# AechPro/rlgym-ppo

Hardware: AMD Instinct MI355X
Metric: ppo_update_samples_per_sec (higher is better)
Workload: dtype f32; 1 GPU; configs[1]: 4096 agents x 128 steps = 524,288-sample buffer, obs 107 f32, 90 discrete actions, 256x3 policy + critic; batch 524,288, minibatch 65,536

## Files before the change

### rlgym_ppo_amd/csrc/api.hip

```cpp
#include "build_id.h"
#include <math.h>
#include <stdarg.h>
#include <string.h>

#include "chain.hpp"

namespace rlppo {

static thread_local char g_err[512] = "";

void set_error(const char *fmt, ...) {
    va_list ap;
    va_start(ap, fmt);
    vsnprintf(g_err, sizeof(g_err), fmt, ap);
    va_end(ap);
}

static int64_t padded_width(int64_t d) {
    const int64_t p16 = round_up(d, 16), p64 = round_up(d, 64);
    return (p64 - p16) * 10 >= p64 ? p16 : p64;
}
static int64_t padded_out(int64_t d) {
    if (d <= 32) return 32;
    if (d <= 64) return 64;
// ... 709 lines not shown
int rlppo_dbg_set(int32_t key, int32_t value) {
    ++g_selection_epoch;
    switch (key) {
        case 1: set_gae_algo(value); return 0;
        case 4: set_two_streams(value); return 0;
        case 19: set_relu_bits(value); return 0;
        case 21: set_gae_spin_limit(value); return 0;
        case 22: set_gae_oversubscribe(value); return 0;
        case 34: set_fused_spin_limit(value); return 0;
        case 35: set_fused_test_hold(value); return 0;
        case 36: set_split_persistent(value); return 0;
        case 23: set_b16_wide_tiles(value); return 0;
        case 24: set_exp_fast_transform(value); return 0;
        case 26: set_fused_gather(value); return 0;
        case 27: g_fused_act = value; return 0;
        case 29: set_paired(value); return 0;
        case 31: set_head_order(value); return 0;
        case 32: set_fold_vhead(value); return 0;
        case 33: set_pair_interleave(value); return 0;
        case 37: set_group_dw(value); return 0;
        case 38: set_tn_group_budget(value); return 0;
        case 40: set_nt_skinny(value); return 0;
        case 41: g_window_mode = value; return 0;
        default: break;
    }
    set_error("dbg_set: unknown key %d", key);
    return RLPPO_ERR_ARG;
}
int64_t rlppo_selection_epoch(void) { return g_selection_epoch; }
const int64_t *rlppo_selection_epoch_ptr(void) { return &g_selection_epoch; }
int rlppo_dbg_count(int32_t key, int64_t delta) {
    RLPPO_CHECK_ARG(key == 6, "dbg_count: key %d (only counter 6 is kept by hosts that replay)", key);
    g_call_counts[CNT_MD_NVEC] += delta;
    return 0;
}
int64_t rlppo_dbg_counter(int32_t key) {
    switch (key) {
        case 0: case 1: case 2: case 3: case 4: case 5: case 6: return g_call_counts[key];
        case 7: return rollout_record_count();
        case 8: case 9: case 10: case 11: case 12: case 13: return g_form_launches[key - 8];
        case 15: return g_call_counts[CNT_CRITIC_ROWS_PASS];
        default: return -1;
    }
}
}
```

### rlgym_ppo_amd/csrc/chain.hip

```cpp
#include "chain.hpp"

namespace rlppo {

int max_pout(const NetLayout &net) {
    int m = 0;
    for (int l = 0; l < net.n_layers; ++l) m = net.L[l].pout > m ? net.L[l].pout : m;
    return m;
}

void x3_layout(const NetLayout &net, X3Layout *o) {
    int64_t off = 0;
    const int last = net.n_layers - 1;
    for (int l = 0; l < net.n_layers; ++l) {
        const LayerLayout &L = net.L[l];
        o->fwd[l] = o->dx[l] = -1;
        if (l >= 1 && l < last && nt_split_ok(L.pout, L.pin)) {
            o->fwd[l] = off;
            off += (int64_t)3 * L.pout * L.pin;
        }
        if (l >= 1 && !(l == last && gemv_head_ok(L.out, L.pin)) && nt_split_ok(L.pin, L.pout)) {
            o->dx[l] = off;
            off += (int64_t)3 * L.pin * L.pout;
        }
    }
// ... 166 lines not shown
            c.f32_valid[l] = true;
        }
        if (rc) return rc;
        x = acts[l];
        xb = actsb[l];
        x_f32 = c.f32_valid[l];
        ldx = L.pout;
    }
    return 0;
}

int layer_backward(Chain &c, int l, bool need_bits) {
    const NetLayout &net = *c.net;
    const int last = net.n_layers - 1;
    const LayerLayout &L = net.L[l];
    const hipStream_t st = c.st;
    const int64_t mb = c.n;
    float *const *acts = c.b.act, *const *dx = c.b.dx;
    const float *dY = l == last ? acts[last] : dx[l];
    const int64_t ld_hy = c.head_folded ? 1 : L.pout;
    const RowSource X = l > 0 ? RowSource{acts[l - 1], net.L[l - 1].pout} : c.in;
    const bool gemv = l == last && l > 0 && gemv_head_ok(L.out, L.pin);
    const size_t floats = tn_layer_floats(net, l, mb, 0);
    int rc = 0;
    if (gemv)
        rc = launch_gemv_dw(st, dY, ld_hy, X.x, X.ld, c.grad + L.off_flat_w, c.grad + L.off_flat_b, L.in, L.pin, mb, c.b.tn, floats);
    else if (c.defer)
        c.defer->add(L, dY, X, c.grad);
    else
        rc = launch_gemm_tn(st, dY, L.pout, L.pout, X.x, X.ld, L.pin, c.grad + L.off_flat_w, c.grad + L.off_flat_b, L.out, L.in, mb,
                            c.b.tn, floats, X.rowtab, X.src_rows);
    if (rc || l == 0) return rc;
    unsigned long long *bits = c.have_bits[l - 1] ? c.b.bits[l - 1] : nullptr;
    rc = -1;
    if (bits && gemv)
        rc = launch_gemv_dx_bits(st, dY, ld_hy, c.w + L.off_w, bits, dx[l - 1], L.pin, L.pin, mb);
    else if (bits) {
        X3Layout xl;
        if (c.x3) x3_layout(net, &xl);
        if (c.x3 && xl.dx[l] >= 0)
            rc = launch_gemm_nt_split(st, dY, L.pout, c.x3 + xl.dx[l], nullptr, dx[l - 1], L.pin, mb, L.pin, L.pout, 1, bits);
        else
            rc = launch_gemm_nt_bits(st, dY, L.pout, c.w + L.off_wt, L.pout, nullptr, dx[l - 1], L.pin, mb, L.pin, L.pout, EPI_MASK, bits);
    }
    if (rc == -1 && need_bits) {
        set_error("paired pass: the output layer's dX needs the bitmask form");
        return RLPPO_ERR_ARG;
    }
    if (rc == -1 && gemv) rc = launch_gemv_dx(st, dY, ld_hy, c.w + L.off_w, acts[l - 1], L.pin, dx[l - 1], L.pin, L.pin, mb, c.hidden_act);
    else if (rc == -1)
        rc = launch_gemm_nt(st, dY, L.pout, c.w + L.off_wt, L.pout, nullptr, acts[l - 1], L.pin, dx[l - 1], L.pin, mb, L.pin, L.pout,
                            hidden_act_dx_epi(c.hidden_act));
    return rc;
}

int backward(Chain &c) {
    for (int l = c.net->n_layers - 1; l >= 0; --l)
        if (int rc = layer_backward(c, l, false)) return rc;
    return 0;
}

int backward_b16(Chain &c) {
    const NetLayout &net = *c.net;
    const hipStream_t st = c.st;
    const int64_t mb = c.n;
    float *const *acts = c.b.act, *const *dx = c.b.dx, *grad = c.grad, *tn_ws = c.b.tn;
    unsigned short *const *actsb = c.b.actb, *const *dxb = c.b.dxb;
    unsigned long long *const *bits = c.b.bits;
    const size_t tn_floats = tn_ws_floats(net, mb, 1);
    const int last = net.n_layers - 1;
    B16Layout bl;
    b16_layout(net, &bl);
    bool dx_f32[RLPPO_MAX_LAYERS] = {};
    int rc = 0;
    auto act_f32 = [&](int l) -> int {
        if (l < 0 || c.f32_valid[l]) return 0;
// ... 86 lines not shown
```

### rlgym_ppo_amd/csrc/chain.hpp

```cpp
#pragma once
#include "common.hpp"

namespace rlppo {

int max_pout(const NetLayout &net);

struct X3Layout {
    int64_t fwd[RLPPO_MAX_LAYERS], dx[RLPPO_MAX_LAYERS], total;
};
void x3_layout(const NetLayout &net, X3Layout *o);
struct B16Layout {
    int64_t w[RLPPO_MAX_LAYERS], wt[RLPPO_MAX_LAYERS], total;
};
void b16_layout(const NetLayout &net, B16Layout *o);

struct RowSource {
    const float *x;
    int64_t ld;
    const unsigned *rowtab = nullptr;
    int64_t src_rows = 0;
};

struct DwList {
    TnProduct p[2 * RLPPO_MAX_LAYERS];
    int n = 0;
    void add(const LayerLayout &L, const float *dY, const RowSource &X, float *grad) {
        TnProduct &q = p[n++];
        q.dY = dY; q.ldy = L.pout; q.ny_valid = L.pout; q.X = X.x; q.ldx = X.ld; q.kx_valid = L.pin;
        q.dW = grad + L.off_flat_w; q.db = grad + L.off_flat_b; q.out = L.out; q.in = L.in;
        q.rowtab = X.rowtab; q.src_rows = X.src_rows;
    }
};

struct NetWs {
    float *act[RLPPO_MAX_LAYERS] = {};
    float *dx[RLPPO_MAX_LAYERS] = {};
    unsigned long long *bits[RLPPO_MAX_LAYERS] = {};
    unsigned short *actb[RLPPO_MAX_LAYERS] = {};
    unsigned short *dxb[RLPPO_MAX_LAYERS] = {};
    float *tn = nullptr;
};

struct Chain {
    hipStream_t st = nullptr;
    const NetLayout *net = nullptr;
    const float *w = nullptr;
    RowSource in = {nullptr, 0};
    const unsigned short *in_b = nullptr;
    int64_t n = 0;
    int out_tanh = 0, hidden_act = ACT_RELU;
    int bf16_operands = 0;
    NetWs b;
    float *grad = nullptr;
    DwList *defer = nullptr;
    const unsigned short *wb16 = nullptr, *x3 = nullptr;
    bool may_fold = false, head_prezeroed = false;
    bool have_bits[RLPPO_MAX_LAYERS] = {}, f32_valid[RLPPO_MAX_LAYERS] = {}, head_folded = false;
};

int forward(Chain &c), backward(Chain &c), forward_b16(Chain &c), backward_b16(Chain &c);
int output_forward(Chain &c, const float *x, int64_t ldx);
int layer_backward(Chain &c, int l, bool need_bits);

size_t tn_layer_floats(const NetLayout &net, int l, int64_t mb, int prec);
size_t tn_ws_floats(const NetLayout &net, int64_t mb, int prec);
void set_fold_vhead(int v);
int get_fold_vhead();

}
```

### rlgym_ppo_amd/csrc/common.hpp

```cpp
#pragma once
#include <hip/hip_runtime.h>
#include <stdint.h>
#include <stdio.h>

#include <atomic>

#include "../../include/rlppo.h"

namespace rlppo {

void set_error(const char *fmt, ...);

#define RLPPO_CHECK_ARG(cond, ...)                \
    do {                                          \
        if (!(cond)) {                            \
            rlppo::set_error(__VA_ARGS__);        \
            return RLPPO_ERR_ARG;                 \
        }                                         \
    } while (0)

#define RLPPO_HIP(expr)                                                                         \
    do {                                                                                        \
        hipError_t e_ = (expr);                                                                 \
        if (e_ != hipSuccess) {                                                                 \
// ... 92 lines not shown
                        int64_t ldc, int64_t M, int N, int nb, int K, int epi);
void set_infer_bf16(int v);
void set_pair_interleave(int v);
void set_nt_skinny(int on);
int get_infer_bf16();
size_t tn_partial_floats(int out, int in, int64_t M);
int launch_gemm_tn(hipStream_t st, const float *dY, int64_t ldy, int ny_valid, const float *X, int64_t ldx, int kx_valid,
                   float *dW, float *db, int out, int in, int64_t M, float *ws, size_t ws_floats, const unsigned *rowtab = nullptr,
                   int64_t src_rows = 0, const TnPair *pair = nullptr);
bool tn_gather_ok(int64_t ldx, int64_t src_rows);
struct TnProduct {
    const float *dY = nullptr;
    int64_t ldy = 0;
    int ny_valid = 0;
    const float *X = nullptr;
    int64_t ldx = 0;
    int kx_valid = 0;
    float *dW = nullptr, *db = nullptr;
    int out = 0, in = 0;
    const unsigned *rowtab = nullptr;
    int64_t src_rows = 0;
};
constexpr int TN_GROUP_MAX = 2 * RLPPO_MAX_LAYERS;
size_t tn_group_floats(const int *outs, const int *ins, int n, int64_t M);
int launch_gemm_tn_group(hipStream_t st, const TnProduct *prods, int n, int64_t M, float *ws, size_t ws_floats);
void set_tn_group_budget(int workgroups);

bool nt_b16_ok(int N, int K, bool hidden);
bool nt_split_ok(int N, int K);
void set_split_persistent(int v);
int launch_pack_split(hipStream_t st, const float *S, int64_t ld, int R, int Cc, unsigned short *planes);
int launch_gemm_nt_split(hipStream_t st, const float *A, int64_t lda, const unsigned short *planes, const float *bias, float *C, int64_t ldc,
                         int64_t M, int N, int K, int mode, unsigned long long *bits);
int launch_gemm_nt_b16(hipStream_t st, const unsigned short *A, int64_t lda, const unsigned short *B, int64_t ldb, const float *bias,
                       float *C, int64_t ldc, unsigned short *Cb, int64_t ldcb, int64_t M, int N, int K, int epi, int mode,
                       unsigned long long *bits);
void set_b16_wide_tiles(int on);
bool tn_b16_ok(int pout, int pin);
int launch_gemm_tn_b16(hipStream_t st, const unsigned short *dY, int64_t ldy, const unsigned short *X, int64_t ldx, float *dW,
                       float *db, int pout, int pin, int out, int in, int64_t M, float *ws, size_t ws_floats);

void set_exp_fast_transform(int on);

bool gemv_head_ok(int out, int kp);
int launch_gemv_fwd(hipStream_t st, const float *x, int64_t ldx, const float *w, const float *b, float *y, int64_t ldy, int64_t n, int kp, int pout);
int launch_gemv_fwd_b16(hipStream_t st, const unsigned short *x, int64_t ldx, const float *w, const float *b, float *y, int64_t ldy,
                        int64_t n, int kp, int pout);
bool thin_head_ok(int out, int kp);
// ... 142 lines not shown
                       int64_t ring_base = 0, int64_t ring_cap = INT64_MAX, const GatherMeta *meta = nullptr);
int launch_gather_meta(hipStream_t st, const int64_t *idx, const float *actions, int act_dim, const float *old_logp,
                       const float *adv, const float *targets, float *g_act, float *g_old, float *g_adv, float *g_tgt, int64_t n,
                       int64_t ring_base, int64_t ring_cap, unsigned *rowtab = nullptr, float *zero_n = nullptr);
struct GatherSide {
    const float *src;
    int64_t ld;
    float *dst;
    int cpr;
};
int launch_gather_rows2(hipStream_t st, const float *src_p, int64_t ld_p, float *dst_p, int width_p, const float *src_c, int64_t ld_c,
                        float *dst_c, int width_c, const int64_t *idx, int64_t n, int64_t ring_base = 0, int64_t ring_cap = INT64_MAX,
                        const GatherMeta *meta = nullptr);
int launch_i64_to_f32(hipStream_t st, const int64_t *src, float *dst, int64_t n);
int launch_learn_report(hipStream_t st, const rlppo_report_args &r);
int launch_signal_words(hipStream_t st, unsigned *words, int count, unsigned value);
int launch_pad_rows(hipStream_t, const void *, int, int64_t, int64_t, int64_t, float *, int64_t, int, float, float);
int launch_pad_rows_vec(hipStream_t, const void *, int, int64_t, int64_t, int64_t, float *, int64_t, const float *, const float *);
int launch_rollout_record(hipStream_t st, const void *rewards, int r_dt, const void *dones, int d_dt, const void *truncated, int t_dt,
                          int64_t n, int64_t t, int64_t T, float *rdt, double *ep_sums, void *state, float *patch);
long long rollout_record_count();
enum LaunchForm { FORM_NT_FEW_ROWS = 0, FORM_NT_TILED, FORM_B16_WIDE, FORM_B16_PERSISTENT, FORM_X3_PERSISTENT, FORM_GEMV_DW_ORDERED, FORM_COUNT };
extern long long g_form_launches[FORM_COUNT];
enum CallCount { CNT_FUSED_ACT = 0, CNT_ACT_CHAIN, CNT_PASS, CNT_PAIRED_PASS, CNT_GATHER_FUSED_PASS, CNT_GROUP_DW, CNT_MD_NVEC, CNT_CRITIC_ROWS_PASS, CNT_COUNT };
extern std::atomic<long long> g_call_counts[CNT_COUNT];
void set_two_streams(int v), set_relu_bits(int v), set_fused_gather(int v), set_paired(int v), set_head_order(int v), set_group_dw(int v);
void set_update_precision(int v);
int get_update_precision();
int launch_obs_scalars(hipStream_t st, const void *mean, const void *m2, int state_f64, long long count, int d, int per_feature,
                       float *mean_v, float *std_v);
int launch_to_trajectory_major(hipStream_t st, const float *S, const float *acts, const float *logp, const float *rdt, int64_t n, int64_t T,
                               int ld, int k, const float *patch, const float *final_rows, float *flat, float *nxt, float *actions,
                               float *log_probs, float *rewards, float *dones, float *truncated);

}
```

### rlgym_ppo_amd/csrc/gemm.hip

```cpp
#include "gemm_detail.hpp"

namespace rlppo {

template <int NB, int EPI, int BKT, bool BITS = false, bool GATHER = false>
__global__ __launch_bounds__(256, BKT == 16 ? 4 : 2) void gemm_nt_dma_kernel(const float *__restrict__ A, unsigned lda_b,
                                                                              const float *__restrict__ B, unsigned ldb_b,
                                                                              const float *__restrict__ bias,
                                                                              const float *__restrict__ mask_src,
                                                                              unsigned ldm_b, float *__restrict__ C,
                                                                              unsigned ldc_b, int64_t M, int K,
                                                                              unsigned long long *__restrict__ bits = nullptr,
                                                                              const unsigned *__restrict__ rowtab = nullptr,
                                                                              unsigned src_rows = 0, NtAlt alt = NtAlt{},
                                                                              NtDot dot = NtDot{}, NtDot dot_alt = NtDot{}) {
    constexpr int BN = NB * 16;
    constexpr int CPR = BKT / 4;
    constexpr int RPW = 64 / CPR;
    constexpr int RPP = 4 * RPW;
    constexpr int A_IT = SBM / RPP, B_IT = BN / RPP;
    constexpr int B_REM = BN % RPP;
    static_assert(B_REM % RPW == 0, "the ragged staging pass must be whole wave instructions");
    __shared__ __attribute__((aligned(16))) float lds[2 * SBM * BKT + 2 * BN * BKT];
    float *As = lds;
    float *Bs = lds + 2 * SBM * BKT;
// ... 913 lines not shown
    TnRedWork w[TN_GROUP_MAX];
};
__global__ __launch_bounds__(256) void tn_reduce_group_kernel(TnRedGroupArgs g) {
    __shared__ __attribute__((aligned(16))) float red[3][64][4];
    __shared__ float dbh[128];
    const int t = blockIdx.y;
    int p = 0;
    for (int i = 1; i < g.n; ++i)
        if (t >= g.w[i].tile_begin) p = i;
    const TnRedWork &w = g.w[p];
    const int nbx = w.geo.ni * w.geo.nj * 4;
    if ((int)blockIdx.x >= nbx) return;
    tn_reduce_tile(w.partial, w.splits, w.tiles_x, w.tiles, w.dW, w.db, w.out, w.in, w.geo, t - w.tile_begin, (int)blockIdx.x, nbx, red, dbh);
}

static int g_tn_group_budget = 0;
constexpr int TN_MAX_CHAIN = 8192;
void set_tn_group_budget(int v) { g_tn_group_budget = v; }
struct TnPlanItem {
    TnGeom g;
    int tiles_x, tiles_y, splits, rows_per_wg, wg_begin;
    size_t partial_off, floats;
};
static int tn_group_plan(const int *outs, const int *ins, int n, int64_t M, int budget, TnPlanItem *it, int *total_wgs, size_t *total_floats) {
    for (int p = 0; p < n; ++p) {
        it[p].g = tn_geometry(outs[p], ins[p]);
        it[p].tiles_x = (int)cdiv(outs[p], it[p].g.bnt());
        it[p].tiles_y = (int)cdiv(ins[p], it[p].g.bkx());
    }
    const int64_t max_splits = cdiv(M, 32);
    auto fill = [&](double t) {
        int64_t wgs = 0;
        for (int p = 0; p < n; ++p) {
            const int blocks = it[p].g.ni * it[p].g.nj;
            int64_t rows = (int64_t)(t / blocks);
            rows = round_up(rows < 32 ? 32 : rows, 32);
            if (g_tn_group_budget <= 0 && rows > TN_MAX_CHAIN) rows = TN_MAX_CHAIN;
            int64_t sp = cdiv(M, rows);
            if (sp > max_splits) sp = max_splits;
            rows = round_up(cdiv(M, sp), 32);
            it[p].rows_per_wg = (int)rows;
            it[p].splits = (int)cdiv(M, rows);
            wgs += round_up((int64_t)it[p].splits * it[p].tiles_x * it[p].tiles_y, 8);
        }
        return wgs;
    };
    for (int rounds = g_tn_group_budget > 0 ? 1 : 2;; ++rounds) {
        const int64_t cap = (int64_t)budget * rounds;
        double lo = 32.0, hi = (double)round_up(M, 32) * 32.0;
        if (fill(lo) <= cap) break;
        for (int i = 0; i < 60; ++i) {
            const double mid = 0.5 * (lo + hi);
            if (fill(mid) > cap) lo = mid; else hi = mid;
        }
        if (fill(hi) <= cap || g_tn_group_budget > 0 || rounds >= 256) break;
    }
    int wg = 0;
    size_t off = 0;
    for (int p = 0; p < n; ++p) {
        it[p].wg_begin = wg;
        wg += (int)round_up((int64_t)it[p].splits * it[p].tiles_x * it[p].tiles_y, 8);
        it[p].partial_off = off;
        it[p].floats = (size_t)it[p].splits * it[p].tiles_x * it[p].tiles_y * (size_t)it[p].g.tile_floats() + (size_t)it[p].splits * it[p].tiles_x * 128;
        off += (it[p].floats + 3) / 4 * 4;
    }
    *total_wgs = wg;
    *total_floats = off;
    return 0;
}
static int tn_group_budget() {
    if (g_tn_group_budget > 0) return g_tn_group_budget;
    int cus = 0;
    if (device_cu_count(&cus) || cus <= 0) cus = 256;
    return 2 * cus;
}
size_t tn_group_floats(const int *outs, const int *ins, int n, int64_t M) {
    if (n <= 0 || M <= 0) return 0;
    size_t total = 0;
    for (int b = 0; b < n; b += TN_GROUP_MAX) {
        TnPlanItem it[TN_GROUP_MAX];
        int wgs = 0;
        size_t f = 0;
        const int m = n - b < TN_GROUP_MAX ? n - b : TN_GROUP_MAX;
        tn_group_plan(outs + b, ins + b, m, M, tn_group_budget(), it, &wgs, &f);
        total = f > total ? f : total;
    }
    return total;
}
int launch_gemm_tn_group(hipStream_t st, const TnProduct *prods, int n, int64_t M, float *ws, size_t ws_floats) {
    if (M <= 0 || n <= 0) return 0;
    for (int b = 0; b < n; b += TN_GROUP_MAX) {
        const int m = n - b < TN_GROUP_MAX ? n - b : TN_GROUP_MAX;
        const TnProduct *pr = prods + b;
        int outs[TN_GROUP_MAX], ins[TN_GROUP_MAX];
        for (int p = 0; p < m; ++p) {
            outs[p] = pr[p].out;
            ins[p] = pr[p].in;
        }
        TnPlanItem it[TN_GROUP_MAX];
        int wgs = 0;
        size_t floats = 0;
        tn_group_plan(outs, ins, m, M, tn_group_budget(), it, &wgs, &floats);
        if (!ws || ws_floats < floats) {
            set_error("gemm_tn_group: workspace %zu < %zu floats", ws ? ws_floats : (size_t)0, floats);
            return RLPPO_ERR_WORKSPACE;
        }
        TnGroupArgs ga{};
        TnRedGroupArgs ra{};
        ga.n = ra.n = m;
        ga.M = M;
        const int64_t lim = (int64_t)1 << 30;
        int tile_begin = 0;
        for (int p = 0; p < m; ++p) {
            const TnProduct &q = pr[p];
            RLPPO_CHECK_ARG(q.dY && q.X && q.dW && q.ny_valid % 4 == 0 && q.kx_valid % 4 == 0 && q.ldy % 4 == 0 && q.ldx % 4 == 0 &&
                                q.ny_valid <= q.ldy && q.kx_valid <= q.ldx && q.out <= q.ny_valid && q.in <= q.kx_valid,
                            "gemm_tn_group: bad shapes (product %d) ny=%d kx=%d ldy=%ld ldx=%ld out=%d in=%d", p, q.ny_valid, q.kx_valid,
                            (long)q.ldy, (long)q.ldx, q.out, q.in);
            RLPPO_CHECK_ARG(((int64_t)it[p].rows_per_wg + TM) * q.ldy * 4 < lim && (q.rowtab || ((int64_t)it[p].rows_per_wg + TM) * q.ldx * 4 < lim),
                            "gemm_tn_group: a leading dimension is too wide for 32-bit tile offsets");
            RLPPO_CHECK_ARG(!q.rowtab || tn_gather_ok(q.ldx, q.src_rows), "gemm_tn_group (gathered rows): unsupported row stride %ld", (long)q.ldx);
            RLPPO_CHECK_ARG(!(q.rowtab && it[p].g.ni == 3), "gemm_tn_group (gathered rows): the 96-row tile has no gathered form");
            TnWork &w = ga.w[p];
            w.dY = q.dY;
            w.X = q.X;
// ... 37 lines not shown
```

### rlgym_ppo_amd/csrc/update.hip

```cpp
#include <math.h>

#include "chain.hpp"

using namespace rlppo;

static int g_two_streams = 1;
static int g_fused_gather = 1;
static int g_update_bf16 = 0;
static int g_group_dw = 1;
static int g_head_order = 1;
static int g_paired = 1;
static int g_relu_bits = 1;
namespace rlppo {
void set_two_streams(int v) { g_two_streams = v; }
void set_fused_gather(int v) { g_fused_gather = v; }
void set_update_precision(int v) { g_update_bf16 = v; }
int get_update_precision() { return g_update_bf16; }
void set_group_dw(int v) { g_group_dw = v; }
void set_head_order(int v) { g_head_order = v; }
void set_paired(int v) { g_paired = v; }
void set_relu_bits(int v) { g_relu_bits = v; }
}

struct SlotBank {
    hipStream_t main[RLPPO_MAX_SLOTS] = {}, side[RLPPO_MAX_SLOTS] = {};
    hipEvent_t ev_fork[RLPPO_MAX_SLOTS] = {}, ev_join[RLPPO_MAX_SLOTS] = {}, ev_slot[RLPPO_MAX_SLOTS] = {}, ev_mid[RLPPO_MAX_SLOTS] = {};
    bool pending[RLPPO_MAX_SLOTS] = {};
};
static SlotBank g_banks[64];
static int slot_bank(SlotBank **bank) {
    int dev = 0;
    RLPPO_HIP(hipGetDevice(&dev));
    RLPPO_CHECK_ARG(dev >= 0 && dev < 64, "device id %d", dev);
    *bank = &g_banks[dev];
    return 0;
}
static int ensure_slot(SlotBank &b, int s) {
    if (!b.side[s]) {
        RLPPO_HIP(hipStreamCreateWithFlags(&b.side[s], hipStreamNonBlocking));
        RLPPO_HIP(hipStreamCreateWithFlags(&b.main[s], hipStreamNonBlocking));
        RLPPO_HIP(hipEventCreateWithFlags(&b.ev_fork[s], hipEventDisableTiming));
        RLPPO_HIP(hipEventCreateWithFlags(&b.ev_join[s], hipEventDisableTiming));
        RLPPO_HIP(hipEventCreateWithFlags(&b.ev_slot[s], hipEventDisableTiming));
        RLPPO_HIP(hipEventCreateWithFlags(&b.ev_mid[s], hipEventDisableTiming));
    }
    return 0;
}
static int order_after(hipStream_t to, hipStream_t from, hipEvent_t ev) {
    RLPPO_HIP(hipEventRecord(ev, from));
    RLPPO_HIP(hipStreamWaitEvent(to, ev, 0));
    return 0;
}

static bool dw_is_gemv(const NetLayout &net, int l) { return l == net.n_layers - 1 && l > 0 && gemv_head_ok(net.L[l].out, net.L[l].pin); }
static size_t tn_region_floats(const NetLayout &pol, const NetLayout &val, int64_t mb, int prec) {
    const size_t chains = tn_ws_floats(pol, mb, prec) + tn_ws_floats(val, mb, prec);
    int outs[2 * RLPPO_MAX_LAYERS], ins[2 * RLPPO_MAX_LAYERS], n = 0;
    for (const NetLayout *net : {&pol, &val})
        for (int l = 0; l < net->n_layers; ++l)
            if (!dw_is_gemv(*net, l)) {
                outs[n] = net->L[l].out;
                ins[n++] = net->L[l].in;
            }
    const size_t group = tn_group_floats(outs, ins, n, mb);
    return chains > group ? chains : group;
}

struct WsPlan {
    NetWs pol, val;
    size_t tn_floats = 0;
    float *states = nullptr;
    float *cstates = nullptr;
    float *g_old = nullptr, *g_adv = nullptr, *g_tgt = nullptr, *g_act = nullptr;
    unsigned *rowtab = nullptr;
    unsigned short *states_b = nullptr;
};
constexpr size_t BITS_PAD_RESERVE = 2, B16_PAD_RESERVE = 4;
static size_t plan_workspace(const NetLayout &pol, const NetLayout &val, int64_t mb, int prec, void *base, WsPlan *w, bool critic_rows = false) {
    const uintptr_t addr = reinterpret_cast<uintptr_t>(base);
    const size_t rows = (size_t)mb;
    size_t off = 0, slack = 0;
    auto take = [&](size_t floats) {
        off += floats;
        return reinterpret_cast<float *>(addr + (off - floats) * sizeof(float));
    };
    auto align = [&](size_t floats, size_t reserve) {
        const size_t pad = (floats - (addr / sizeof(float) + off) % floats) % floats;
        off += pad;
// ... 28 lines not shown
        for (int i = 0; i < 2; ++i)
            for (int l = 0; l + 1 < nets[i]->n_layers; ++l) el += 2 * (size_t)nets[i]->L[l].pout;
        unsigned short *hb = reinterpret_cast<unsigned short *>(take((el * rows + 1) / 2));
        auto take16 = [&](size_t n) {
            hb += n;
            return hb - n;
        };
        w->states_b = take16(rows * pol.L[0].pin);
        for (int i = 0; i < 2; ++i)
            for (int l = 0; l + 1 < nets[i]->n_layers; ++l) ws[i]->actb[l] = take16(rows * nets[i]->L[l].pout);
        for (int i = 0; i < 2; ++i)
            for (int l = 0; l + 1 < nets[i]->n_layers; ++l) ws[i]->dxb[l] = take16(rows * nets[i]->L[l].pout);
    }
    return off + slack;
}

static int resolve_precision(int32_t precision, int *mode) {
    RLPPO_CHECK_ARG(precision >= 0 && precision <= 3, "update precision %d (0 = process default, 1 = fp32, 2 = bf16 mixed precision, 3 = split-bf16 products)", precision);
    *mode = precision == RLPPO_PRECISION_DEFAULT ? g_update_bf16 : precision - 1;
    return 0;
}

constexpr int64_t PAIRED_MIN_ROWS = 262144;
static bool twin_ok(const NetLayout &p, const NetLayout &v, int64_t mb) {
    if (p.n_layers != v.n_layers || p.n_layers < 2) return false;
    for (int l = 0; l + 1 < p.n_layers; ++l) {
        const LayerLayout &a = p.L[l], &b = v.L[l];
        if (a.in != b.in || a.out != b.out || a.pin != b.pin || a.pout != b.pout) return false;
        if (a.pout % 128 != 0 || a.pin % 16 != 0 || nt_bits_floats(mb, a.pout) == 0) return false;
    }
    return true;
}

constexpr int64_t FUSED_GATHER_MIN_ROWS = 262144;
static void first_layer_rows(const rlppo_minibatch_args &a, const rlppo_critic_rows *critic, const NetLayout &pol, const NetLayout &val, int prec,
                             const WsPlan &w, bool plain, RowSource rows[2]) {
    const float *vx = critic ? critic->states : a.states;
    const int64_t vld = critic ? critic->ld_states : a.ld_states;
    rows[0] = RowSource{w.states, pol.L[0].pin};
    rows[1] = critic ? RowSource{w.cstates, val.L[0].pin} : rows[0];
    if (plain) return;
    const int64_t src_rows = a.ring_cap > 0 ? a.ring_cap : a.n_rows;
    auto gather_form = [&](const NetLayout &n, int64_t ld) {
        return n.n_layers > 1 && nt_gather_ok(ld, src_rows, n.L[0].pout, n.L[0].pin) && tn_gather_ok(ld, src_rows) &&
               !(n.L[0].out > 64 && n.L[0].out <= 96 && !(n.L[0].in > 96 && n.L[0].in <= 112));
    };
    if (prec != 1 && (g_fused_gather == 2 || (g_fused_gather == 1 && a.mb >= FUSED_GATHER_MIN_ROWS)) && src_rows > 0 &&
        gather_form(pol, a.ld_states) && gather_form(val, vld)) {
        rows[0] = RowSource{a.states, a.ld_states, w.rowtab, src_rows};
        rows[1] = RowSource{vx, vld, w.rowtab, src_rows};
    }
}

struct Pass {
    const rlppo_minibatch_args *a;
    NetLayout pol, val;
    int64_t mb;
    int prec;
    int64_t ring_base, ring_cap;
    WsPlan w;
    const rlppo_critic_rows *critic = nullptr;
    RowSource rows[2];
    LossCfg cfg;
    MdSpec md;
    bool md_general = false;
    const DiagHead *diag = nullptr;
    const float *pol_w, *val_w;
    hipStream_t st, side;
    DwList *defer;
    int pol_act = ACT_RELU, val_act = ACT_RELU;
    bool plain = false;
};

static Chain pass_chain(const Pass &p, bool critic) {
    const rlppo_minibatch_args &a = *p.a;
    const unsigned short *image = reinterpret_cast<const unsigned short *>(critic ? a.val_wb16 : a.pol_wb16);
    Chain c;
    c.st = critic ? p.side : p.st;
    c.net = critic ? &p.val : &p.pol;
    c.w = critic ? p.val_w : p.pol_w;
    c.in = p.rows[critic ? 1 : 0];
    c.in_b = p.w.states_b;
    c.n = p.mb;
    c.out_tanh = !critic && a.head == RLPPO_HEAD_GAUSSIAN;
    c.hidden_act = critic ? p.val_act : p.pol_act;
    c.b = critic ? p.w.val : p.w.pol;
    if (p.plain)
        for (auto &bits : c.b.bits) bits = nullptr;
    c.grad = critic ? a.val_grad : a.pol_grad;
    c.defer = p.defer;
    c.wb16 = p.prec == 1 ? image : nullptr;
    c.x3 = p.prec == 2 ? image : nullptr;
    c.may_fold = c.head_prezeroed = critic && !p.plain;
    return c;
}

static LossCfg loss_cfg(const rlppo_minibatch_args &a) {
    LossCfg c;
    c.clip = a.clip_range;
    c.clip_lo = (float)(1.0 - (double)a.clip_range);
    c.clip_hi = (float)(1.0 + (double)a.clip_range);
    c.ent_coef = a.ent_coef;
    c.mb_ratio = a.mb_ratio;
    c.inv_mb = 1.0f / (float)a.mb;
    c.var_m = a.var_m;
    c.var_b = a.var_b;
    c.adv_norm = a.adv_norm;
    c.vclip = a.value_clip;
    c.kl_slots = a.kl_slots;
    c.stop_word = a.stop_word;
    return c;
}

// ... 77 lines not shown
        }
        rc = launch_gemm_nt_bits(st, xp, ldx, p.pol_w + Lp.off_w, Lp.pin, p.pol_w + Lp.off_b, w.pol.act[l], Lp.pout, mb, Lp.pout, Lp.pin,
                                 EPI_BIAS_RELU, w.pol.bits[l], l == 0 ? rows.rowtab : nullptr, rows.src_rows, &alt,
                                 fold_here ? dots : nullptr);
        if (rc) {
            if (rc == -1) set_error("paired pass: a hidden layer does not have the bitmask form");
            return rc == -1 ? RLPPO_ERR_ARG : rc;
        }
        cp.have_bits[l] = cv.have_bits[l] = true;
        xp = w.pol.act[l];
        xv = w.val.act[l];
        ldx = Lp.pout;
    }
    if (hs != st) {
        rc = order_after(hs, st, bk.ev_fork[slot]);
        if (rc) return rc;
    }
    if (!fold_v) {
        rc = output_forward(cv, xv, ldx);
        if (rc) return rc;
    }
    rc = launch_value_loss(hs, vout, ldv, w.g_tgt, w.g_adv, mb, p.cfg, a.stats);
    if (rc) return rc;
    const bool ordered = g_head_order && hs != st;
    if (!ordered) {
        rc = layer_backward(cv, H, true);
        if (rc) return rc;
    }
    rc = output_forward(cp, xp, ldx);
    if (rc) return rc;
    rc = policy_loss(st, p);
    if (rc) return rc;
    if (ordered) {
        rc = order_after(hs, st, bk.ev_mid[slot]);
        if (rc) return rc;
        rc = layer_backward(cv, H, true);
        if (rc) return rc;
    }
    rc = layer_backward(cp, H, true);
    if (rc) return rc;
    if (hs != st) {
        rc = order_after(st, hs, bk.ev_join[slot]);
        if (rc) return rc;
    }
    for (int l = H - 1; l >= 0; --l) {
        const LayerLayout &Lp = pol.L[l], &Lv = val.L[l];
        const RowSource Xp = l > 0 ? RowSource{w.pol.act[l - 1], pol.L[l - 1].pout} : rows;
        const RowSource Xv = l > 0 ? RowSource{w.val.act[l - 1], val.L[l - 1].pout} : rows;
        if (p.defer) {
            p.defer->add(Lp, w.pol.dx[l], Xp, a.pol_grad);
            p.defer->add(Lv, w.val.dx[l], Xv, a.val_grad);
        } else {
            TnPair pr;
            pr.dY = w.val.dx[l];
            pr.X = Xv.x;
            pr.dW = a.val_grad + Lv.off_flat_w;
            pr.db = a.val_grad + Lv.off_flat_b;
            pr.ws = w.val.tn;
            rc = launch_gemm_tn(st, w.pol.dx[l], Lp.pout, Lp.pout, Xp.x, Xp.ld, Lp.pin, a.pol_grad + Lp.off_flat_w, a.pol_grad + Lp.off_flat_b,
                                Lp.out, Lp.in, mb, w.pol.tn, tn_layer_floats(pol, l, mb, 0), Xp.rowtab, Xp.src_rows, &pr);
            if (rc) return rc;
        }
        if (l == 0) break;
        NtAlt alt;
        alt.A = w.val.dx[l];
        alt.B = p.val_w + Lv.off_wt;
        alt.C = w.val.dx[l - 1];
        alt.bits = w.val.bits[l - 1];
        rc = launch_gemm_nt_bits(st, w.pol.dx[l], Lp.pout, p.pol_w + Lp.off_wt, Lp.pout, nullptr, w.pol.dx[l - 1], Lp.pin, mb, Lp.pin,
                                 Lp.pout, EPI_MASK, w.pol.bits[l - 1], nullptr, 0, &alt);
        if (rc) return rc == -1 ? RLPPO_ERR_ARG : rc;
    }
    return 0;
}

static int two_chain_pass(const Pass &p) {
    Chain val = pass_chain(p, true), pol = pass_chain(p, false);
    const bool b16 = p.prec == 1;
    for (Chain *c : {&val, &pol})
        if (int rc = b16 ? forward_b16(*c) : forward(*c)) return rc;
    const int vlast = p.val.n_layers - 1;
    const int64_t ldv = val.head_folded ? 1 : p.val.L[vlast].pout;
    int rc = launch_value_loss(p.side, p.w.val.act[vlast], ldv, p.w.g_tgt, p.w.g_adv, p.mb, p.cfg, p.a->stats);
    if (rc) return rc;
    rc = policy_loss(p.st, p);
    if (rc) return rc;
    for (Chain *c : {&val, &pol})
        if ((rc = b16 ? backward_b16(*c) : backward(*c))) return rc;
    return 0;
}

static int ppo_minibatch(void *stream, const rlppo_minibatch_args *a, const int32_t *md_nvec, int32_t md_heads, const DiagHead *diag,
                         int pol_act, int val_act, const rlppo_critic_rows *critic = nullptr, const float *vnorm = nullptr) {
    RLPPO_CHECK_ARG(a != nullptr, "ppo_minibatch: null args");
    Pass p;
    p.a = a;
// ... 74 lines not shown
        if (rc) return rc;
        p.md_general = true;
        RLPPO_CHECK_ARG(p.md.S == n_out, "multi-discrete head: md_nvec sums to %d, but the policy has %d outputs", p.md.S, n_out);
        RLPPO_CHECK_ARG(a->act_dim == p.md.H, "multi-discrete head: act_dim=%d, but md_heads=%d", a->act_dim, p.md.H);
    } else if (a->head == RLPPO_HEAD_MULTIDISCRETE)
        RLPPO_CHECK_ARG(n_out == 21 && a->act_dim == 8, "multi-discrete head: needs 21 outputs and act_dim 8");
    RLPPO_CHECK_ARG(p.prec != 1 || (a->pol_packed_r && a->val_packed_r && a->pol_wb16 && a->val_wb16),
                    "ppo_minibatch: the bf16 update precision needs the rlppo_net_pack_bf16 images of both networks (pol_packed_r / val_packed_r / pol_wb16 / val_wb16)");
    RLPPO_CHECK_ARG(p.prec != 2 || (a->pol_wb16 && a->val_wb16),
                    "ppo_minibatch: the split-bf16 update precision needs the rlppo_net_pack_x3 images of both networks (pol_wb16 / val_wb16)");
    rc = ring_window("ppo_minibatch", a->ring_base, a->ring_cap, &p.ring_base, &p.ring_cap);
    if (rc) return rc;
    const int slot = a->slot;
    RLPPO_CHECK_ARG(slot >= 0 && slot < RLPPO_MAX_SLOTS, "ppo_minibatch: slot %d not in [0, %d)", slot, RLPPO_MAX_SLOTS);

    first_layer_rows(*a, critic, pol, val, p.prec, p.w, p.plain, p.rows);
    const bool twin = p.prec == 0 && !p.plain && !critic && (g_paired == 2 || (g_paired == 1 && mb >= PAIRED_MIN_ROWS)) && twin_ok(pol, val, mb);
    p.cfg = loss_cfg(*a);
    p.cfg.vnorm = vnorm;
    p.pol_w = p.prec == 1 ? a->pol_packed_r : a->pol_packed;
    p.val_w = p.prec == 1 ? a->val_packed_r : a->val_packed;
    DwList dws;
    p.defer = (g_group_dw && p.prec != 1) ? &dws : nullptr;

    SlotBank *bank = nullptr;
    rc = slot_bank(&bank);
    if (rc) return rc;
    SlotBank &bk = *bank;
    rc = ensure_slot(bk, slot);
    if (rc) return rc;
    const hipStream_t caller = (hipStream_t)stream;
    p.st = caller;
    if (slot > 0) {
        p.st = bk.main[slot];
        rc = order_after(p.st, caller, bk.ev_slot[slot]);
        if (rc) return rc;
        bk.pending[slot] = true;
    }
    rc = gather(p);
    if (rc) return rc;
    p.side = p.st;
    if (g_two_streams) {
        p.side = bk.side[slot];
        rc = order_after(p.side, p.st, bk.ev_fork[slot]);
        if (rc) return rc;
    }
    ++g_call_counts[CNT_PASS];
    if (twin) ++g_call_counts[CNT_PAIRED_PASS];
    if (p.rows[0].rowtab) ++g_call_counts[CNT_GATHER_FUSED_PASS];
    if (critic) ++g_call_counts[CNT_CRITIC_ROWS_PASS];
    rc = twin ? paired_pass(p, bk, slot) : two_chain_pass(p);
    if (rc) return rc;
    if (!twin && p.side != p.st) {
        rc = order_after(p.st, p.side, bk.ev_join[slot]);
        if (rc) return rc;
    }
    if (p.defer && dws.n) {
        ++g_call_counts[CNT_GROUP_DW];
        rc = launch_gemm_tn_group(p.st, dws.p, dws.n, mb, p.w.pol.tn, p.w.tn_floats);
    }
    return rc;
}

static DiagHead diag_head(const float *log_std, float *log_std_grad, void *scratch, size_t scratch_bytes) {
    return DiagHead{log_std, log_std_grad, reinterpret_cast<double *>(scratch), scratch_bytes};
}

extern "C" {

size_t rlppo_minibatch_workspace_bytes_for(const int32_t *pol_dims, int32_t pol_layers, const int32_t *val_dims, int32_t val_layers,
                                           int64_t mb, int32_t precision) {
    NetLayout pol, val;
    int prec = 0;
    if (make_layout(pol_dims, pol_layers, &pol) || make_layout(val_dims, val_layers, &val) || resolve_precision(precision, &prec)) return 0;
    WsPlan unused;
    return plan_workspace(pol, val, mb > 0 ? mb : 0, prec, nullptr, &unused) * sizeof(float) + 256;
}
size_t rlppo_minibatch_workspace_bytes_critic(const int32_t *pol_dims, int32_t pol_layers, const int32_t *val_dims, int32_t val_layers,
                                              int64_t mb, int32_t precision) {
    NetLayout pol, val;
    int prec = 0;
    if (make_layout(pol_dims, pol_layers, &pol) || make_layout(val_dims, val_layers, &val) || resolve_precision(precision, &prec)) return 0;
// ... 79 lines not shown
```

Before: 62.90 million samples/s.

## Launch critic penultimate-layer weight gradient early on side stream to overlap policy backward

For large minibatches the critic's penultimate-layer dW product is pulled out of the deferred grouped TN GEMM. It is launched on the side stream right after the critic head's dX, so it can overlap with the policy chain's backward work on the main stream. The grouped-GEMM planner gains a workspace-fit mode that shrinks split counts so the early product and the remaining group both fit the shared tn workspace. This adds extra event synchronisation and a tail join. The reduced split parallelism and workspace sharing between concurrently running kernels could contend.

Result: no change. 63.06 million samples/s (median of 6 runs) (+0.3%).

```diff
diff --git a/rlgym_ppo_amd/csrc/api.hip b/rlgym_ppo_amd/csrc/api.hip
--- a/rlgym_ppo_amd/csrc/api.hip
+++ b/rlgym_ppo_amd/csrc/api.hip
@@ -755,6 +755,7 @@
         case 38: set_tn_group_budget(value); return 0;
         case 40: set_nt_skinny(value); return 0;
         case 41: g_window_mode = value; return 0;
+        case 42: set_early_dw(value); return 0;
         default: break;
     }
     set_error("dbg_set: unknown key %d", key);
@@ -773,6 +774,7 @@
         case 7: return rollout_record_count();
         case 8: case 9: case 10: case 11: case 12: case 13: return g_form_launches[key - 8];
         case 15: return g_call_counts[CNT_CRITIC_ROWS_PASS];
+        case 17: return g_call_counts[CNT_EARLY_DW];
         default: return -1;
     }
 }
diff --git a/rlgym_ppo_amd/csrc/chain.hip b/rlgym_ppo_amd/csrc/chain.hip
--- a/rlgym_ppo_amd/csrc/chain.hip
+++ b/rlgym_ppo_amd/csrc/chain.hip
@@ -212,12 +212,14 @@
     const RowSource X = l > 0 ? RowSource{acts[l - 1], net.L[l - 1].pout} : c.in;
     const bool gemv = l == last && l > 0 && gemv_head_ok(L.out, L.pin);
     const size_t floats = tn_layer_floats(net, l, mb, 0);
+    const bool early_head = gemv && c.defer && c.early_layer == l - 1;
     int rc = 0;
-    if (gemv)
-        rc = launch_gemv_dw(st, dY, ld_hy, X.x, X.ld, c.grad + L.off_flat_w, c.grad + L.off_flat_b, L.in, L.pin, mb, c.b.tn, floats);
-    else if (c.defer)
-        c.defer->add(L, dY, X, c.grad);
-    else
+    if (gemv) {
+        if (!early_head)
+            rc = launch_gemv_dw(st, dY, ld_hy, X.x, X.ld, c.grad + L.off_flat_w, c.grad + L.off_flat_b, L.in, L.pin, mb, c.b.tn, floats);
+    } else if (c.defer) {
+        if (l != c.early_layer) c.defer->add(L, dY, X, c.grad);
+    } else
         rc = launch_gemm_tn(st, dY, L.pout, L.pout, X.x, X.ld, L.pin, c.grad + L.off_flat_w, c.grad + L.off_flat_b, L.out, L.in, mb,
                             c.b.tn, floats, X.rowtab, X.src_rows);
     if (rc || l == 0) return rc;
@@ -241,7 +243,16 @@
     else if (rc == -1)
         rc = launch_gemm_nt(st, dY, L.pout, c.w + L.off_wt, L.pout, nullptr, acts[l - 1], L.pin, dx[l - 1], L.pin, mb, L.pin, L.pout,
                             hidden_act_dx_epi(c.hidden_act));
-    return rc;
+    if (rc || !early_head) return rc;
+    if (c.ev_dx) RLPPO_HIP(hipEventRecord(c.ev_dx, st));
+    const int e = l - 1, k = c.defer->n_early;
+    c.defer->add(net.L[e], dx[e], e > 0 ? RowSource{acts[e - 1], net.L[e - 1].pout} : c.in, c.grad, true);
+    if (c.early_now) {
+        ++g_call_counts[CNT_EARLY_DW];
+        rc = launch_gemm_tn_group(st, c.defer->early + k, 1, mb, c.early_ws, c.early_floats, true);
+        if (rc) return rc;
+    }
+    return launch_gemv_dw(st, dY, ld_hy, X.x, X.ld, c.grad + L.off_flat_w, c.grad + L.off_flat_b, L.in, L.pin, mb, c.b.tn, floats);
 }
 
 int backward(Chain &c) {
diff --git a/rlgym_ppo_amd/csrc/chain.hpp b/rlgym_ppo_amd/csrc/chain.hpp
--- a/rlgym_ppo_amd/csrc/chain.hpp
+++ b/rlgym_ppo_amd/csrc/chain.hpp
@@ -22,10 +22,10 @@
 };
 
 struct DwList {
-    TnProduct p[2 * RLPPO_MAX_LAYERS];
-    int n = 0;
-    void add(const LayerLayout &L, const float *dY, const RowSource &X, float *grad) {
-        TnProduct &q = p[n++];
+    TnProduct p[2 * RLPPO_MAX_LAYERS], early[2];
+    int n = 0, n_early = 0;
+    void add(const LayerLayout &L, const float *dY, const RowSource &X, float *grad, bool is_early = false) {
+        TnProduct &q = is_early ? early[n_early++] : p[n++];
         q.dY = dY; q.ldy = L.pout; q.ny_valid = L.pout; q.X = X.x; q.ldx = X.ld; q.kx_valid = L.pin;
         q.dW = grad + L.off_flat_w; q.db = grad + L.off_flat_b; q.out = L.out; q.in = L.in;
         q.rowtab = X.rowtab; q.src_rows = X.src_rows;
@@ -53,6 +53,11 @@
     NetWs b;
     float *grad = nullptr;
     DwList *defer = nullptr;
+    int early_layer = -1;
+    bool early_now = false;
+    float *early_ws = nullptr;
+    size_t early_floats = 0;
+    hipEvent_t ev_dx = nullptr;
     const unsigned short *wb16 = nullptr, *x3 = nullptr;
     bool may_fold = false, head_prezeroed = false;
     bool have_bits[RLPPO_MAX_LAYERS] = {}, f32_valid[RLPPO_MAX_LAYERS] = {}, head_folded = false;
diff --git a/rlgym_ppo_amd/csrc/common.hpp b/rlgym_ppo_amd/csrc/common.hpp
--- a/rlgym_ppo_amd/csrc/common.hpp
+++ b/rlgym_ppo_amd/csrc/common.hpp
@@ -138,8 +138,8 @@
     int64_t src_rows = 0;
 };
 constexpr int TN_GROUP_MAX = 2 * RLPPO_MAX_LAYERS;
-size_t tn_group_floats(const int *outs, const int *ins, int n, int64_t M);
-int launch_gemm_tn_group(hipStream_t st, const TnProduct *prods, int n, int64_t M, float *ws, size_t ws_floats);
+size_t tn_group_floats(const int *outs, const int *ins, int n, int64_t M, size_t max_floats = 0);
+int launch_gemm_tn_group(hipStream_t st, const TnProduct *prods, int n, int64_t M, float *ws, size_t ws_floats, bool fit = false);
 void set_tn_group_budget(int workgroups);
 
 bool nt_b16_ok(int N, int K, bool hidden);
@@ -328,9 +328,9 @@
 long long rollout_record_count();
 enum LaunchForm { FORM_NT_FEW_ROWS = 0, FORM_NT_TILED, FORM_B16_WIDE, FORM_B16_PERSISTENT, FORM_X3_PERSISTENT, FORM_GEMV_DW_ORDERED, FORM_COUNT };
 extern long long g_form_launches[FORM_COUNT];
-enum CallCount { CNT_FUSED_ACT = 0, CNT_ACT_CHAIN, CNT_PASS, CNT_PAIRED_PASS, CNT_GATHER_FUSED_PASS, CNT_GROUP_DW, CNT_MD_NVEC, CNT_CRITIC_ROWS_PASS, CNT_COUNT };
+enum CallCount { CNT_FUSED_ACT = 0, CNT_ACT_CHAIN, CNT_PASS, CNT_PAIRED_PASS, CNT_GATHER_FUSED_PASS, CNT_GROUP_DW, CNT_MD_NVEC, CNT_CRITIC_ROWS_PASS, CNT_EARLY_DW, CNT_COUNT };
 extern std::atomic<long long> g_call_counts[CNT_COUNT];
-void set_two_streams(int v), set_relu_bits(int v), set_fused_gather(int v), set_paired(int v), set_head_order(int v), set_group_dw(int v);
+void set_two_streams(int v), set_relu_bits(int v), set_fused_gather(int v), set_paired(int v), set_head_order(int v), set_group_dw(int v), set_early_dw(int v);
 void set_update_precision(int v);
 int get_update_precision();
 int launch_obs_scalars(hipStream_t st, const void *mean, const void *m2, int state_f64, long long count, int d, int per_feature,
diff --git a/rlgym_ppo_amd/csrc/gemm.hip b/rlgym_ppo_amd/csrc/gemm.hip
--- a/rlgym_ppo_amd/csrc/gemm.hip
+++ b/rlgym_ppo_amd/csrc/gemm.hip
@@ -959,7 +959,8 @@
     int tiles_x, tiles_y, splits, rows_per_wg, wg_begin;
     size_t partial_off, floats;
 };
-static int tn_group_plan(const int *outs, const int *ins, int n, int64_t M, int budget, TnPlanItem *it, int *total_wgs, size_t *total_floats) {
+static int tn_group_plan(const int *outs, const int *ins, int n, int64_t M, int budget, TnPlanItem *it, int *total_wgs, size_t *total_floats,
+                         size_t max_floats = 0) {
     for (int p = 0; p < n; ++p) {
         it[p].g = tn_geometry(outs[p], ins[p]);
         it[p].tiles_x = (int)cdiv(outs[p], it[p].g.bnt());
@@ -992,6 +993,25 @@
         }
         if (fill(hi) <= cap || g_tn_group_budget > 0 || rounds >= 256) break;
     }
+    auto floats_of = [&](int p) {
+        return ((size_t)it[p].splits * it[p].tiles_x * it[p].tiles_y * (size_t)it[p].g.tile_floats() + (size_t)it[p].splits * it[p].tiles_x * 128 + 3) / 4 * 4;
+    };
+    for (int tries = 0; max_floats && tries < 24; ++tries) {
+        size_t total = 0;
+        int64_t wgs = 0;
+        for (int p = 0; p < n; ++p) {
+            total += floats_of(p);
+            wgs += round_up((int64_t)it[p].splits * it[p].tiles_x * it[p].tiles_y, 8);
+        }
+        if (total <= max_floats) break;
+        const int64_t cap = (int64_t)((double)wgs * (double)max_floats / (double)total * 0.97);
+        double lo = 32.0, hi = (double)round_up(M, 32) * 32.0;
+        for (int i = 0; i < 60; ++i) {
+            const double mid = 0.5 * (lo + hi);
+            if (fill(mid) > cap) lo = mid; else hi = mid;
+        }
+        fill(hi);
+    }
     int wg = 0;
     size_t off = 0;
     for (int p = 0; p < n; ++p) {
@@ -1011,7 +1031,7 @@
     if (device_cu_count(&cus) || cus <= 0) cus = 256;
     return 2 * cus;
 }
-size_t tn_group_floats(const int *outs, const int *ins, int n, int64_t M) {
+size_t tn_group_floats(const int *outs, const int *ins, int n, int64_t M, size_t max_floats) {
     if (n <= 0 || M <= 0) return 0;
     size_t total = 0;
     for (int b = 0; b < n; b += TN_GROUP_MAX) {
@@ -1019,12 +1039,12 @@
         int wgs = 0;
         size_t f = 0;
         const int m = n - b < TN_GROUP_MAX ? n - b : TN_GROUP_MAX;
-        tn_group_plan(outs + b, ins + b, m, M, tn_group_budget(), it, &wgs, &f);
+        tn_group_plan(outs + b, ins + b, m, M, tn_group_budget(), it, &wgs, &f, max_floats);
         total = f > total ? f : total;
     }
     return total;
 }
-int launch_gemm_tn_group(hipStream_t st, const TnProduct *prods, int n, int64_t M, float *ws, size_t ws_floats) {
+int launch_gemm_tn_group(hipStream_t st, const TnProduct *prods, int n, int64_t M, float *ws, size_t ws_floats, bool fit) {
     if (M <= 0 || n <= 0) return 0;
     for (int b = 0; b < n; b += TN_GROUP_MAX) {
         const int m = n - b < TN_GROUP_MAX ? n - b : TN_GROUP_MAX;
@@ -1037,7 +1057,7 @@
         TnPlanItem it[TN_GROUP_MAX];
         int wgs = 0;
         size_t floats = 0;
-        tn_group_plan(outs, ins, m, M, tn_group_budget(), it, &wgs, &floats);
+        tn_group_plan(outs, ins, m, M, tn_group_budget(), it, &wgs, &floats, fit ? ws_floats : 0);
         if (!ws || ws_floats < floats) {
             set_error("gemm_tn_group: workspace %zu < %zu floats", ws ? ws_floats : (size_t)0, floats);
             return RLPPO_ERR_WORKSPACE;
diff --git a/rlgym_ppo_amd/csrc/update.hip b/rlgym_ppo_amd/csrc/update.hip
--- a/rlgym_ppo_amd/csrc/update.hip
+++ b/rlgym_ppo_amd/csrc/update.hip
@@ -9,6 +9,7 @@
 static int g_update_bf16 = 0;
 static int g_group_dw = 1;
 static int g_head_order = 1;
+static int g_early_dw = 1;
 static int g_paired = 1;
 static int g_relu_bits = 1;
 namespace rlppo {
@@ -19,12 +20,14 @@
 void set_group_dw(int v) { g_group_dw = v; }
 void set_head_order(int v) { g_head_order = v; }
 void set_paired(int v) { g_paired = v; }
+void set_early_dw(int v) { g_early_dw = v; }
 void set_relu_bits(int v) { g_relu_bits = v; }
 }
 
 struct SlotBank {
     hipStream_t main[RLPPO_MAX_SLOTS] = {}, side[RLPPO_MAX_SLOTS] = {};
     hipEvent_t ev_fork[RLPPO_MAX_SLOTS] = {}, ev_join[RLPPO_MAX_SLOTS] = {}, ev_slot[RLPPO_MAX_SLOTS] = {}, ev_mid[RLPPO_MAX_SLOTS] = {};
+    hipEvent_t ev_tail[RLPPO_MAX_SLOTS] = {};
     bool pending[RLPPO_MAX_SLOTS] = {};
 };
 static SlotBank g_banks[64];
@@ -43,6 +46,7 @@
         RLPPO_HIP(hipEventCreateWithFlags(&b.ev_join[s], hipEventDisableTiming));
         RLPPO_HIP(hipEventCreateWithFlags(&b.ev_slot[s], hipEventDisableTiming));
         RLPPO_HIP(hipEventCreateWithFlags(&b.ev_mid[s], hipEventDisableTiming));
+        RLPPO_HIP(hipEventCreateWithFlags(&b.ev_tail[s], hipEventDisableTiming));
     }
     return 0;
 }
@@ -53,17 +57,31 @@
 }
 
 static bool dw_is_gemv(const NetLayout &net, int l) { return l == net.n_layers - 1 && l > 0 && gemv_head_ok(net.L[l].out, net.L[l].pin); }
-static size_t tn_region_floats(const NetLayout &pol, const NetLayout &val, int64_t mb, int prec) {
+static size_t tn_region_floats(const NetLayout &pol, const NetLayout &val, int64_t mb, int prec, int *early = nullptr) {
     const size_t chains = tn_ws_floats(pol, mb, prec) + tn_ws_floats(val, mb, prec);
-    int outs[2 * RLPPO_MAX_LAYERS], ins[2 * RLPPO_MAX_LAYERS], n = 0;
+    const int vlast = val.n_layers - 1;
+    int outs[2 * RLPPO_MAX_LAYERS], ins[2 * RLPPO_MAX_LAYERS], n = 0, at = -1;
     for (const NetLayout *net : {&pol, &val})
         for (int l = 0; l < net->n_layers; ++l)
             if (!dw_is_gemv(*net, l)) {
+                if (net == &val && l == vlast - 1) at = n;
                 outs[n] = net->L[l].out;
                 ins[n++] = net->L[l].in;
             }
     const size_t group = tn_group_floats(outs, ins, n, mb);
-    return chains > group ? chains : group;
+    const size_t region = chains > group ? chains : group;
+    if (!early) return region;
+    *early = -1;
+    if (prec == 1 || mb <= 0 || !dw_is_gemv(val, vlast) || dw_is_gemv(pol, pol.n_layers - 1)) return region;
+    if (tn_group_floats(outs + at, ins + at, 1, mb, region) > region) return region;
+    for (int i = at; i + 1 < n; ++i) outs[i] = outs[i + 1], ins[i] = ins[i + 1];
+    if (tn_group_floats(outs, ins, n - 1, mb, region) <= region) *early = vlast - 1;
+    return region;
+}
+static int early_dw_layer(const NetLayout &pol, const NetLayout &val, int64_t mb, int prec) {
+    int e = -1;
+    tn_region_floats(pol, val, mb, prec, &e);
+    return e;
 }
 
 struct WsPlan {
@@ -138,6 +156,12 @@
 }
 
 constexpr int64_t PAIRED_MIN_ROWS = 262144;
+constexpr int64_t EARLY_DW_MIN_ROWS = 262144;
+static int early_dw_mode(int64_t mb) {
+    if (g_early_dw == 0) return 1;
+    if (g_early_dw == 2 || (g_early_dw == 1 && mb >= EARLY_DW_MIN_ROWS)) return 2;
+    return 0;
+}
 static bool twin_ok(const NetLayout &p, const NetLayout &v, int64_t mb) {
     if (p.n_layers != v.n_layers || p.n_layers < 2) return false;
     for (int l = 0; l + 1 < p.n_layers; ++l) {
@@ -184,6 +208,8 @@
     const float *pol_w, *val_w;
     hipStream_t st, side;
     DwList *defer;
+    int early = -1;
+    bool early_now = false;
     int pol_act = ACT_RELU, val_act = ACT_RELU;
     bool plain = false;
 };
@@ -205,6 +231,12 @@
         for (auto &bits : c.b.bits) bits = nullptr;
     c.grad = critic ? a.val_grad : a.pol_grad;
     c.defer = p.defer;
+    if (critic && p.early >= 0) {
+        c.early_layer = p.early;
+        c.early_now = p.early_now;
+        c.early_ws = p.w.pol.tn;
+        c.early_floats = p.w.tn_floats;
+    }
     c.wb16 = p.prec == 1 ? image : nullptr;
     c.x3 = p.prec == 2 ? image : nullptr;
     c.may_fold = c.head_prezeroed = critic && !p.plain;
@@ -328,7 +360,9 @@
     }
     rc = launch_value_loss(hs, vout, ldv, w.g_tgt, w.g_adv, mb, p.cfg, a.stats);
     if (rc) return rc;
-    const bool ordered = g_head_order && hs != st;
+    const bool early = cv.early_layer >= 0 && cv.early_now && hs != st;
+    if (early) cv.ev_dx = bk.ev_join[slot];
+    const bool ordered = (early ? g_head_order == 2 : g_head_order != 0) && hs != st;
     if (!ordered) {
         rc = layer_backward(cv, H, true);
         if (rc) return rc;
@@ -345,7 +379,9 @@
     }
     rc = layer_backward(cp, H, true);
     if (rc) return rc;
-    if (hs != st) {
+    if (early)
+        RLPPO_HIP(hipStreamWaitEvent(st, bk.ev_join[slot], 0));
+    else if (hs != st) {
         rc = order_after(st, hs, bk.ev_join[slot]);
         if (rc) return rc;
     }
@@ -355,7 +391,7 @@
         const RowSource Xv = l > 0 ? RowSource{w.val.act[l - 1], val.L[l - 1].pout} : rows;
         if (p.defer) {
             p.defer->add(Lp, w.pol.dx[l], Xp, a.pol_grad);
-            p.defer->add(Lv, w.val.dx[l], Xv, a.val_grad);
+            if (l != cv.early_layer) p.defer->add(Lv, w.val.dx[l], Xv, a.val_grad);
         } else {
             TnPair pr;
             pr.dY = w.val.dx[l];
@@ -377,7 +413,7 @@
                                  Lp.pout, EPI_MASK, w.pol.bits[l - 1], nullptr, 0, &alt);
         if (rc) return rc == -1 ? RLPPO_ERR_ARG : rc;
     }
-    return 0;
+    return early ? order_after(st, hs, bk.ev_tail[slot]) : 0;
 }
 
 static int two_chain_pass(const Pass &p) {
@@ -498,6 +534,8 @@
     p.val_w = p.prec == 1 ? a->val_packed_r : a->val_packed;
     DwList dws;
     p.defer = (g_group_dw && p.prec != 1) ? &dws : nullptr;
+    p.early = p.defer && !p.plain && early_dw_mode(mb) ? early_dw_layer(pol, val, mb, p.prec) : -1;
+    p.early_now = early_dw_mode(mb) == 2;
 
     SlotBank *bank = nullptr;
     rc = slot_bank(&bank);
@@ -533,7 +571,9 @@
     }
     if (p.defer && dws.n) {
         ++g_call_counts[CNT_GROUP_DW];
-        rc = launch_gemm_tn_group(p.st, dws.p, dws.n, mb, p.w.pol.tn, p.w.tn_floats);
+        rc = launch_gemm_tn_group(p.st, dws.p, dws.n, mb, p.w.pol.tn, p.w.tn_floats, p.early >= 0);
+        if (rc == 0 && dws.n_early && !p.early_now)
+            rc = launch_gemm_tn_group(p.st, dws.early, dws.n_early, mb, p.w.pol.tn, p.w.tn_floats, true);
     }
     return rc;
 }
```
